# c-f-h/pyiga

Hardware: AMD Instinct MI355X
Metric: assembled elements/sec (3D p=4, 128^3 spans) + HBM-roofline %; 1/2/4/8 GPU (higher is better)
Workload: dtype f64

## Files before the change

### pyiga_amd/csrc/fused3.hip

```cpp
#include "igx_internal.h"
#include "fused_common.h"
#include <algorithm>
#include <cstdio>
#include <cstdlib>
#include <cstring>
#include <vector>

#ifndef BF3_FIXED_PASS
#define BF3_FIXED_PASS 1
#endif
#ifndef BF3_MASS_AXSYM
#define BF3_MASS_AXSYM 1
#endif
#ifndef BF3_MASS_STW
#define BF3_MASS_STW 1
#endif
#ifndef BF3_MASS_STW_QMAX
#define BF3_MASS_STW_QMAX 3
#endif

namespace igx {

template <int P1, int P2, int Q, int NLG, int NRO, int NCW, int SYM> struct BF3Geom {
    static constexpr int P1_ = P1, P2_ = P2, Q_ = Q;
    static constexpr int p1 = P1 - 1, p2 = P2 - 1, W1 = 2 * P1 - 1, W2 = 2 * P2 - 1, TL = 64 * NLG;
    static constexpr int NSET = SYM == 2 ? 2 : 1;
    static constexpr int QS = Q + (Q % 2 == 0 ? 1 : 0), NSP = (TL + Q - 1) / Q;
    static constexpr int TLP = TL + NSP * (QS - Q);
    static constexpr int VS = Q * P2 * 2 + ((Q * P2 * 2) % 4 == 2 ? 0 : 2), NV2 = NSP * VS;
    static constexpr int LS = NRO * TLP + 2;
    static constexpr int NRING = p1 * (p1 + 1) / 2 + p1;
    static constexpr int NRL = NRING + P1;
    static constexpr int T0 = p2 * (p2 + 1) / 2;
    static constexpr int NEL = 2 * p2 * W2;
    static constexpr int off_sets() { return (W1 * LS + 1) & ~1; }
    static constexpr int off_v2(int R) { return (off_sets() + NSET * (NRL * R * W2 + 2) + 1) & ~1; }
    static constexpr int off_etab(int R) { return off_v2(R) + NV2; }
    static constexpr int lds_doubles(int R) { return off_etab(R) + NEL * 2; }
    static constexpr int rmax()
    {
        int R = TL / Q - p2;
        while (R > 1 && lds_doubles(R) * 8 > 160 * 1024) --R;
        return R;
    }
    static constexpr int RMAX = rmax();
    static constexpr int RW = RMAX * W2;
    static constexpr int SETSZ = NRL * RW + 2;
    static constexpr int OFF_PAD = NRL * RW;
    static constexpr int roff(int d) { return RW * ((d - 1) * (d + 2) / 2); }
    static constexpr int OFF_CUR = NRING * RW;
    static constexpr int OFF_SETS = off_sets(), OFF_V2 = off_v2(RMAX), OFF_ETAB = off_etab(RMAX);
    static constexpr int LDS_BYTES = lds_doubles(RMAX) * 8;
    static constexpr int NSUB = (RW + 63) / 64;
    static constexpr int npc(int pl) { return (RMAX + pl - p2 - 1) / (pl - p2); }
    static constexpr int npass(int pl) { return (W1 * npc(pl) + 64 / pl - 1) / (64 / pl); }
    static constexpr int pick()
    {
        int best = 64;
        const int cand[4] = {64, 32, 21, 16};
        for (int i = 1; i < 4; ++i)
            if (cand[i] > 2 * p2 && npass(cand[i]) < npass(best)) best = cand[i];
        return best;
    }
    static constexpr int PL = pick(), PPP = 64 / PL, NPC = npc(PL), RP = PL - p2;
};

struct BF3Blk {
    int i0, j0, diag0, c0i, c0j, cj0, ci0, rlo, rhi, row_lo, nrows, stD, stT, ne;
    long long S12;
};

typedef int bf3_v4i __attribute__((ext_vector_type(4)));

template <class Gm> struct BF3Row {
    int on, l0, c1, rp1d, sub1, sub2, sub3, sub4, sub5;
    __device__ __forceinline__ static BF3Row of(const BFArgs &A, const BF3Blk &B, const int t)
    {
        cip rp1 = (cip)A.rp1, jlo1 = (cip)A.jlo1, jhi1 = (cip)A.jhi1;
        constexpr int p1 = Gm::p1, RW = Gm::RW;
        BF3Row r;
        const int d = t - 1;
        r.on = d >= B.rlo && d < B.rhi;
        const int dc = min(max(d, 0), A.N1 - 1);
        const int jl1 = jlo1[dc];
        r.c1 = jhi1[dc] - jl1; r.l0 = p1 - (dc - jl1);
        r.rp1d = rp1[dc];
        r.sub1 = Gm::roff(1) + (int)((unsigned)dc % 2u) * RW; r.sub2 = Gm::roff(2) + (int)((unsigned)dc % 3u) * RW;
        r.sub3 = Gm::roff(3) + (int)((unsigned)dc % 4u) * RW; r.sub4 = Gm::roff(4) + (int)((unsigned)dc % 5u) * RW;
        r.sub5 = Gm::roff(5) + (int)((unsigned)dc % 6u) * RW;
        return r;
    }
    __device__ __forceinline__ int line_off(const int l) const
    {
        constexpr int p1 = Gm::p1;
        int o = Gm::OFF_CUR + (l - p1) * Gm::RW;
        o = l == p1 - 1 ? sub1 : o;
        if (p1 >= 2) o = l == p1 - 2 ? sub2 : o;
        if (p1 >= 3) o = l == p1 - 3 ? sub3 : o;
        if (p1 >= 4) o = l == p1 - 4 ? sub4 : o;
        if (p1 >= 5) o = l == p1 - 5 ? sub5 : o;
        return o;
    }
    __device__ __forceinline__ bool line_ok(const int l) const { return l < Gm::W1 && l >= l0 && l - l0 < c1; }
};
__device__ __forceinline__ __amdgpu_buffer_rsrc_t bf3_rs(double *ptr, const int len) { return __builtin_amdgcn_make_buffer_rsrc((void *)ptr, (short)0, len, 0x00020000); }

template <class Gm, int NS, int ROT, int NH, int SYM, bool TR>
struct BF3Store {
    static constexpr int P1 = Gm::P1_, W1 = Gm::W1, W2 = Gm::W2, p2 = Gm::p2, NSUB = Gm::NSUB, RW = Gm::RW;
    static constexpr int JMAX = (W1 + NS - 1) / NS, NST = NSUB * JMAX, NSET = SYM == 2 ? 2 : 1;
    using Row = BF3Row<Gm>;
    int rrv[NSUB];
    int ev[TR ? NSUB : 1];
    int lane8, lanec, inv;
    double *pD, *pT;
    int nD, nT;

    __device__ __forceinline__ void init(const BFArgs &A, const BF3Blk &B, const int , const int lane)
    {
        cip rp0 = (cip)A.rp0;
        lane8 = lane * 8;
        lanec = min((NSUB - 1) * 64 + lane, RW - 1) - (NSUB - 1) * 64;
        if constexpr (TR) {
            pD = A.data + ((long long)rp0[B.i0] * B.S12 - A.nnz_off); nD = B.stD ? (int)((long long)B.c0i * B.S12 * 8) : 0;
            pT = A.data + ((long long)rp0[B.j0] * B.S12 - A.nnz_off); nT = B.stT ? (int)((long long)B.c0j * B.S12 * 8) : 0;
            inv = 2 * (int)A.S2 + 1;
#pragma unroll
            for (int c = 0; c < NSUB; ++c) {
                const int q = c * 64 + lane, rr = q / W2, i2 = B.row_lo + rr;
                const bool ok = q < RW && rr < B.nrows && i2 >= p2 && i2 <= A.N2 - 1 - p2;
                rrv[c] = ok ? W2 * i2 - Gm::T0 : inv;
                ev[c] = 8 * (q - rr * W2);
            }
            return;
        }
        const long long shift = (long long)W2 * B.row_lo - Gm::T0;
        const long long lenD = ((long long)B.c0i * B.S12 - shift) * 8, lenT = ((long long)B.c0j * B.S12 - shift) * 8;
        pD = A.data + ((long long)rp0[B.i0] * B.S12 - A.nnz_off + shift); nD = B.stD ? (int)lenD : 0;
        pT = A.data + ((long long)rp0[B.j0] * B.S12 - A.nnz_off + shift); nT = B.stT ? (int)lenT : 0;
        const int c0min = min(B.c0i, B.c0j);
        inv = (int)(max(lenD, lenT) / (8 * max(c0min * 2 - 1, 1))) + 1;
#pragma unroll
        for (int c = 0; c < NSUB; ++c) {
            const int q = c * 64 + lane, rr = q / W2, i2 = B.row_lo + rr;
            const bool ok = q < RW && rr < B.nrows && i2 >= p2 && i2 <= A.N2 - 1 - p2;
            rrv[c] = ok ? W2 * i2 - Gm::T0 : inv;
        }
    }
    __device__ __forceinline__ static int line_of(const int sw, const int c, const int j) { return (int)((unsigned)(sw + ROT * c) % (unsigned)NS) + NS * j; }

    template <int X>
    __device__ __forceinline__ void move_row(double *sets, double *dump, const int sw, const int lane, const Row &r, double *ptr, const int len, const int sK, const int soff0)
    {
        int lb_ = lane, lc_ = lanec;
        asm volatile("" : "+v"(lb_), "+v"(lc_));
        double *bs = sets + X * Gm::SETSZ + lb_, *bc = sets + X * Gm::SETSZ + (NSUB - 1) * 64 + lc_;
        double v[NST];
#pragma unroll
        for (int c = 0; c < NSUB; ++c)
#pragma unroll
            for (int j = 0; j < JMAX; ++j) {
                const int l = line_of(sw, c, j);
                double *src = (c == NSUB - 1 ? bc : bs + c * 64) + r.line_off(min(l, W1 - 1));
                v[c * JMAX + j] = *src;
                if (NH >= 2) {
                    double *cl = (rrv[c] != inv && l < W1) ? src : dump;
                    *cl = 0.0;
                }
            }
#ifdef BF3_NOSTORE
        return;
#endif
        int voff[NSUB];
#pragma unroll
        for (int c = 0; c < NSUB; ++c) {
            if constexpr (TR) voff[c] = (int)(__umul24((unsigned)rrv[c], (unsigned)sK) + __umul24((unsigned)ev[c], (unsigned)r.c1));
            else voff[c] = (int)__umul24((unsigned)rrv[c], (unsigned)sK) + lane8;
            asm volatile("" : "+v"(voff[c]));
        }
#pragma unroll
        for (int c = 0; c < NSUB; ++c)
#pragma unroll
            for (int j = 0; j < JMAX; ++j) {
                const int l = line_of(sw, c, j);
                if constexpr (TR) bf2_buffer_store(bf3_rs(ptr, r.line_ok(l) ? len : 0), voff[c], soff0 + 8 * l, v[c * JMAX + j]);
                else bf2_buffer_store(bf3_rs(ptr, r.line_ok(l) ? len : 0), voff[c] + c * 512, soff0 + 8 * W2 * l, v[c * JMAX + j]);
            }
    }
    __device__ __forceinline__ void fetch(const BFArgs &A, const BF3Blk &B, double *sets, double *dump, const int t, const int sw, const int lane)
    {
        const Row r = Row::of(A, B, t);
        if constexpr (TR) {
            const int sD = 8 * B.c0i * (int)A.S1, sT = 8 * B.c0j * (int)A.S1;
            const int oD = 8 * (W2 * (B.c0i * r.rp1d + B.cj0 * r.c1) - r.l0), oT = 8 * (W2 * (B.c0j * r.rp1d + B.ci0 * r.c1) - r.l0);
            move_row<0>(sets, dump, sw, lane, r, pD, r.on ? nD : 0, sD, oD);
            if (NSET == 2) move_row<1>(sets, dump, sw, lane, r, pT, r.on ? nT : 0, sT, oT);
            if (SYM == 3) move_row<0>(sets, dump, sw, lane, r, pT, r.on ? nT : 0, sT, oT);
            return;
        }
        move_row<0>(sets, dump, sw, lane, r, pD, r.on ? nD : 0, 8 * (B.c0i * r.c1 - 1), 8 * ((int)((long long)B.c0i * A.S2) * r.rp1d + W2 * (B.cj0 * r.c1 - r.l0)));
        if (NSET == 2)
            move_row<1>(sets, dump, sw, lane, r, pT, r.on ? nT : 0, 8 * (B.c0j * r.c1 - 1), 8 * ((int)((long long)B.c0j * A.S2) * r.rp1d + W2 * (B.ci0 * r.c1 - r.l0)));
        if (SYM == 3)
            move_row<0>(sets, dump, sw, lane, r, pT, r.on ? nT : 0, 8 * (B.c0j * r.c1 - 1), 8 * ((int)((long long)B.c0j * A.S2) * r.rp1d + W2 * (B.ci0 * r.c1 - r.l0)));
    }
};

template <int NR, int NLG, int NQ> struct BF3DenseSplit {
    static constexpr int NA = (NR - 2) * NLG, NB = NLG;
    static constexpr int ka() { if (NA == 0) return 0; int k = 1; while (NA * k + NB * ((3 * k + 1) / 2) < NQ) ++k; return k; }
    static constexpr int KA = ka(), KB = NA == 0 ? (NQ + NB - 1) / NB : (3 * KA + 1) / 2;
    static constexpr int QB = NA * KA < NQ ? NA * KA : NQ;
};
constexpr int BF3_FAR = 0x7f000000;
template <class Gm, int NH, int SYM, int K, int QLO, int QHI, int QSTR, bool TR>
struct BF3StoreDense {
    static constexpr int p1 = Gm::p1, p2 = Gm::p2, W1 = Gm::W1, W2 = Gm::W2, WW = W1 * W2, RW = Gm::RW, NSET = SYM == 2 ? 2 : 1;
    using Row = BF3Row<Gm>;
    double svD[K], svT[NSET == 2 ? K : 1];
    int pk[K];
    int lane8;
    double *pD, *pT;
    long long nD, nT;

    __device__ __forceinline__ void init(const BFArgs &A, const BF3Blk &B, const int sw, const int lane)
    {
        cip rp0 = (cip)A.rp0;
        lane8 = lane * 8;
        pD = A.data + ((long long)rp0[B.i0] * B.S12 - A.nnz_off); nD = B.stD ? (long long)B.c0i * B.S12 * 8 : 0;
        pT = A.data + ((long long)rp0[B.j0] * B.S12 - A.nnz_off); nT = B.stT ? (long long)B.c0j * B.S12 * 8 : 0;
#pragma unroll
        for (int k = 0; k < K; ++k) {
            svD[k] = 0.0;
            if (NSET == 2) svT[k] = 0.0;
            const int qi = QLO + sw + QSTR * k;
            const int q = qi * 64 + lane, rr = q / WW, rem = q - rr * WW, l = rem / W2, e = rem - l * W2, i2 = B.row_lo + rr;
            const bool ok = qi < QHI && q < Gm::RMAX * WW && rr < B.nrows && i2 >= p2 && i2 <= A.N2 - 1 - p2;
            pk[k] = ok ? (4 * l) | ((rr * W2 + e) << 6) | (rr << 18) : (int)(0x80000000u | 60u);
        }
    }

    __device__ __forceinline__ void fetch(const BFArgs &A, const BF3Blk &B, double *sets, double *dump, const int t, const int sw, const int lane)
    {
        const Row r = Row::of(A, B, t);
        int lv = Gm::OFF_CUR + (lane - p1) * RW;
        lv = lane == p1 - 1 ? r.sub1 : lv;
        if (p1 >= 2) lv = lane == p1 - 2 ? r.sub2 : lv;
        if (p1 >= 3) lv = lane == p1 - 3 ? r.sub3 : lv;
        if (p1 >= 4) lv = lane == p1 - 4 ? r.sub4 : lv;
        if (p1 >= 5) lv = lane == p1 - 5 ? r.sub5 : lv;
        lv = lane == 15 ? Gm::OFF_PAD : lv;
#pragma unroll
        for (int k = 0; k < K; ++k) {
            int pkk = pk[k];
            asm volatile("" : "+v"(pkk));
            const int lo = __builtin_amdgcn_ds_bpermute(pkk & 60, lv) + ((pkk >> 6) & 0xfff);
            double *src = sets + lo;
            svD[k] = *src;
#ifndef BF3_NOCLEAR
            if (NH >= 2) *src = 0.0;
#endif
            if (NSET == 2) {
                double *srcT = src + Gm::SETSZ;
                svT[k] = *srcT;
#ifndef BF3_NOCLEAR
                if (NH >= 2) *srcT = 0.0;
#endif
            }
        }
        (void)dump;
    }

    __device__ __forceinline__ void issue(const BFArgs &A, const BF3Blk &B, const int t, const int sw)
    {
#ifdef BF3_NOSTORE
        return;
#endif
        const Row r = Row::of(A, B, t);
        if constexpr (TR) {
            const long long rowc = (long long)W2 * B.row_lo - Gm::T0;
            const long long shD = (long long)B.c0i * A.S1 * rowc + (long long)W2 * (B.c0i * r.rp1d + B.cj0 * r.c1) - r.l0;
            const long long shT = (long long)B.c0j * A.S1 * rowc + (long long)W2 * (B.c0j * r.rp1d + B.ci0 * r.c1) - r.l0;
            const __amdgpu_buffer_rsrc_t dD = bf3_rs(pD + shD, r.on ? (int)max(nD - shD * 8, 0LL) : 0);
            const __amdgpu_buffer_rsrc_t dT = bf3_rs(pT + shT, r.on ? (int)max(nT - shT * 8, 0LL) : 0);
            const int dlD = 8 * W2 * (B.c0i * (int)A.S1 - r.c1), dlT = 8 * W2 * (B.c0j * (int)A.S1 - r.c1), c18 = 8 * r.c1;
            const int lane = lane8 >> 3;
            const int offl = (unsigned)(lane - r.l0) < (unsigned)r.c1 ? lane8 : BF3_FAR;
#pragma unroll
            for (int k = 0; k < K; ++k) {
                int pkk = pk[k];
                asm volatile("" : "+v"(pkk));
                const int rr = (pkk >> 18) & 0xff;
                const int q8 = __builtin_amdgcn_ds_bpermute(pkk & 60, offl) + (int)__mul24((pkk >> 6) & 0xfff, c18);
                bf2_buffer_store(dD, (int)__mul24(rr, dlD) + q8, 0, svD[k]);
                if (NSET == 2) bf2_buffer_store(dT, (int)__mul24(rr, dlT) + q8, 0, svT[k]);
                if (SYM == 3) bf2_buffer_store(dT, (int)__mul24(rr, dlT) + q8, 0, svD[k]);
            }
            return;
        }
        const int cD = B.c0i * r.c1, cT = B.c0j * r.c1;
        const long long rowc = (long long)W2 * B.row_lo - Gm::T0;
        const long long shD = (long long)B.c0i * A.S2 * r.rp1d + cD * rowc + W2 * (B.cj0 * r.c1 - r.l0);
        const __amdgpu_buffer_rsrc_t dD = bf3_rs(pD + shD, r.on ? (int)max(nD - shD * 8, 0LL) : 0);
        const int dlD = 8 * W2 * (cD - W1);
        const long long shT = (long long)B.c0j * A.S2 * r.rp1d + cT * rowc + W2 * (B.ci0 * r.c1 - r.l0);
        const __amdgpu_buffer_rsrc_t dT = bf3_rs(pT + shT, r.on ? (int)max(nT - shT * 8, 0LL) : 0);
        const int dlT = 8 * W2 * (cT - W1);
        const int lane = lane8 >> 3;
        const int offl = (unsigned)(lane - r.l0) < (unsigned)r.c1 ? 0 : BF3_FAR;
#pragma unroll
        for (int k = 0; k < K; ++k) {
            int pkk = pk[k];
            asm volatile("" : "+v"(pkk));
            const int rr = (pkk >> 18) & 0xff;
            const int q8 = __builtin_amdgcn_ds_bpermute(pkk & 60, offl) + ((QLO + sw + QSTR * k) * 512 + lane8);
            bf2_buffer_store(dD, (int)__mul24(rr, dlD) + q8, 0, svD[k]);
            if (NSET == 2) bf2_buffer_store(dT, (int)__mul24(rr, dlT) + q8, 0, svT[k]);
            if (SYM == 3) bf2_buffer_store(dT, (int)__mul24(rr, dlT) + q8, 0, svD[k]);
        }
    }
};

template <class Gm, int NCW, int NH, int SYM, bool TR>
__device__ __forceinline__ void bf3_edge_rows(const BFArgs &A, const BF3Blk &B, double *sets, const bf3_v4i *etab, const int t, const int cw, const int lane)
{
    constexpr int W1 = Gm::W1, W2 = Gm::W2;
    if (B.ne == 0) return;
    cip rp0 = (cip)A.rp0;
    const BF3Row<Gm> r = BF3Row<Gm>::of(A, B, t);
    const long long shift = (long long)W2 * B.row_lo - Gm::T0;
    static_assert(SYM != 3 || NH == 1, "per-axis symmetry: the second store reads the rows again (no halves, no clears)");
#pragma unroll
    for (int X = 0; X < (SYM == 3 ? 2 : Gm::NSET); ++X) {
        if (X == 0 ? !B.stD : !B.stT) continue;
        const int c0x = X == 0 ? B.c0i : B.c0j, cx = X == 0 ? B.cj0 : B.ci0;
        double *px = A.data + ((long long)rp0[X == 0 ? B.i0 : B.j0] * B.S12 - A.nnz_off + (TR ? 0 : shift));
        const int nx = (int)(((long long)c0x * B.S12 - (TR ? 0 : shift)) * 8);
        const unsigned sA = TR ? (unsigned)(c0x * r.rp1d + cx * r.c1) : (unsigned)(c0x * r.c1);
        const unsigned sC = (unsigned)(8 * c0x * (int)A.S1);
        const int soffr = TR ? 0 : 8 * (int)((long long)c0x * A.S2) * r.rp1d;
        for (int l = (int)((unsigned)(cw + NCW - X) % (unsigned)NCW); l < W1; l += NCW) {
            const unsigned sB = TR ? (unsigned)r.c1 : (unsigned)max(cx * r.c1 + l - r.l0, 0);
            const __amdgpu_buffer_rsrc_t dsc = bf3_rs(px, (r.on && r.line_ok(l)) ? nx : 0);
            double *lb = sets + (SYM == 3 ? 0 : X) * Gm::SETSZ + r.line_off(l);
            for (int ch = 0; ch * 64 < B.ne * W2; ++ch) {
                const bf3_v4i e = etab[min(ch * 64 + lane, Gm::NEL - 1)];
                const bool ok = ch * 64 + lane < Gm::NEL && e.w != BF2_OOB;
                double *src = lb + e.x;
                const double v = *src;
                if (NH >= 2 && ok) *src = 0.0;
                int off = (int)(__umul24(sA, (unsigned)e.y) + __umul24(sB, (unsigned)e.z));
                if constexpr (TR) off += (int)__umul24(sC, (unsigned)e.w) + 8 * (l - r.l0);
                else off += e.w;
                bf2_buffer_store(dsc, ok ? off : BF2_OOB, soffr, v);
            }
        }
    }
}

struct BF3SweepCtx { const BF3Blk *B; double *sets, *dump; int sw, tlp; };
template <int P1, int Q, int D, int MASK, int RI, int NA, int NLG, class StoreT, bool STW, bool MULT>
__device__ __forceinline__ void bf3_sweeper(const BFArgs &A, const int r0, const int g2l, const int g2, const int s_begin, const int t_sw, const int d_begin,
                                            const int rhi, double *lines, const int LS, const BF3SweepCtx &sc)
{
    constexpr BFRole R = bf_role(MASK, RI);
    constexpr int p1 = P1 - 1;
    constexpr bool ST = STW && (RI >= 1 || bf_nroles(MASK) == 1);
    const int slane = threadIdx.x & 63;
    StoreT store;
    if constexpr (ST) store.init(A, *sc.B, sc.sw, slane);
    BF_STAMP_DECL
    __builtin_amdgcn_s_setprio(BF2_PRIO_S);
    cdp V1 = (cdp)A.V1;
    cip fa1 = (cip)A.fa1;
    double acc[P1][P1];
#pragma unroll
    for (int a = 0; a < P1; ++a)
#pragma unroll
        for (int b = 0; b < P1; ++b) acc[a][b] = 0.0;
    __amdgpu_buffer_rsrc_t rsrc[4][NA];
    int urs[4][NA];
    const int voff = g2 * 8;
#pragma unroll
    for (int t1 = 0; t1 < 4; ++t1)
#pragma unroll
        for (int i = 0; i < NA; ++i) {
            urs[t1][i] = A.rs[R.y][t1][i] * 8;
            rsrc[t1][i] = bf2_rsrc(A.sp[R.y][t1][i] + (long long)r0 * A.ss[R.y][t1][i] - (long long)A.gmid_lo * A.rs[R.y][t1][i]);
        }
    auto ld = [&](const int t1, const int i, const int row) {
#ifdef BF3_NOLOAD
        return (double)(row + t1);
#else
        return bf2_buffer_load(rsrc[t1][i], voff, row * urs[t1][i]);
#endif
    };
    static_assert(Q % D == 0, "k_bf3: the prefetch ring must divide the span");
    double kv[D][4][NA];
    {
        const int s = min(s_begin, max(t_sw - 1, 0));
#pragma unroll
        for (int l = 0; l < D; ++l)
#pragma unroll
            for (int t1 = 0; t1 < 4; ++t1)
                if (R.has[t1])
#pragma unroll
                    for (int i = 0; i < NA; ++i) kv[l][t1][i] = ld(t1, i, s * Q + l);
    }
    auto flush = [&](const bool zero) {
        double *ln = lines + RI * sc.tlp + g2l;
#pragma unroll
        for (int a = 0; a < P1; ++a) ln[a * LS] = acc[a][0];
#pragma unroll
        for (int a = 1; a < P1; ++a) ln[(p1 + a) * LS] = acc[0][a];
#pragma unroll
        for (int a = 0; a < P1 - 1; ++a)
#pragma unroll
            for (int b = 0; b < P1 - 1; ++b) acc[a][b] = acc[a + 1][b + 1];
        if (zero) {
#pragma unroll
            for (int a = 0; a < P1; ++a) { acc[a][P1 - 1] = 0.0; acc[P1 - 1][a] = 0.0; }
        }
    };
    auto sweep_span = [&](const int s) __attribute__((always_inline)) {
        const int tn = min(s + 1, t_sw - 1);
        cdp cf = V1 + (size_t)s * Q * P1 * 2;
        double v[P1][2];
#pragma unroll
        for (int b = 0; b < P1; ++b) { v[b][0] = cf[2 * b]; v[b][1] = cf[2 * b + 1]; }
#pragma unroll
        for (int l = 0; l < Q; ++l) {
            double vn[P1][2];
            const int ln_ = l + 1 < Q ? l + 1 : l;
#pragma unroll
            for (int b = 0; b < P1; ++b) { vn[b][0] = cf[(ln_ * P1 + b) * 2]; vn[b][1] = cf[(ln_ * P1 + b) * 2 + 1]; }
            double kt[4] = {0.0, 0.0, 0.0, 0.0};
#pragma unroll
            for (int t1 = 0; t1 < 4; ++t1)
                if (R.has[t1]) {
                    kt[t1] = kv[l % D][t1][0];
                    if constexpr (NA == 2) kt[t1] += kv[l % D][t1][1];
#pragma unroll
                    for (int i = 0; i < NA; ++i) kv[l % D][t1][i] = ld(t1, i, l + D < Q ? s * Q + l + D : tn * Q + l + D - Q);
                }
            if (R.shape == 1) {
#pragma unroll
                for (int b = 0; b < P1; ++b) {
                    double w;
                    if (R.has[2 * R.f] && R.has[2 * R.f + 1]) w = fma(v[b][1], kt[2 * R.f + 1], v[b][0] * kt[2 * R.f]);
                    else if (R.has[2 * R.f]) w = v[b][0] * kt[2 * R.f];
                    else w = v[b][1] * kt[2 * R.f + 1];
#pragma unroll
                    for (int a = 0; a < P1; ++a) {
                        if (l == 0 && (a == P1 - 1 || b == P1 - 1)) acc[a][b] = v[a][R.f] * w;
                        else acc[a][b] = fma(v[a][R.f], w, acc[a][b]);
                    }
                }
            } else {
                constexpr int tu_first = (R.has[0] || R.has[2]) ? 0 : 1;
#pragma unroll
                for (int tu = 0; tu < 2; ++tu) {
                    if (!(R.has[tu] || R.has[tu + 2])) continue;
#pragma unroll
                    for (int a = 0; a < P1; ++a) {
                        double c;
                        if (R.has[tu] && R.has[tu + 2]) c = fma(v[a][1], kt[tu + 2], v[a][0] * kt[tu]);
                        else if (R.has[tu]) c = v[a][0] * kt[tu];
                        else c = v[a][1] * kt[tu + 2];
#pragma unroll
                        for (int b = 0; b < P1; ++b) {
                            if (l == 0 && tu == tu_first && (a == P1 - 1 || b == P1 - 1)) acc[a][b] = v[b][tu] * c;
                            else acc[a][b] = fma(v[b][tu], c, acc[a][b]);
                        }
                    }
                }
            }
#pragma unroll
            for (int a = 0; a < P1; ++a)
#pragma unroll
                for (int b = 0; b < P1; ++b) asm volatile("" : "+v"(acc[a][b]));
#pragma unroll
            for (int b = 0; b < P1; ++b) { v[b][0] = vn[b][0]; v[b][1] = vn[b][1]; }
        }
    };
    if constexpr (!MULT) {
        int d = d_begin;
        for (; d < t_sw; ++d) {
            bar_lds();
            if constexpr (ST) store.issue(A, *sc.B, d - 1, sc.sw);
            sweep_span(d);
            bar_lds();
            flush(d + 1 >= t_sw);
            if constexpr (ST) store.fetch(A, *sc.B, sc.sets, sc.dump, d, sc.sw, slane);
        }
        for (; d < rhi; ++d) {
            bar_lds();
            if constexpr (ST) store.issue(A, *sc.B, d - 1, sc.sw);
            bar_lds(); flush(true);
            if constexpr (ST) store.fetch(A, *sc.B, sc.sets, sc.dump, d, sc.sw, slane);
        }
    } else {
        int s = s_begin;
        for (int d = d_begin; d < rhi; ++d) {
            bar_lds();
            if constexpr (ST) store.issue(A, *sc.B, d - 1, sc.sw);
            if (s < t_sw && fa1[s] == d) { sweep_span(s); ++s; }
            bar_lds();
            flush(true);
            if constexpr (ST) store.fetch(A, *sc.B, sc.sets, sc.dump, d, sc.sw, slane);
        }
    }
    {
        bar_lds();
        if constexpr (ST) store.issue(A, *sc.B, rhi - 1, sc.sw);
        bar_lds();
        if constexpr (ST) store.fetch(A, *sc.B, sc.sets, sc.dump, rhi, sc.sw, slane);
    }
    if constexpr (ST) store.issue(A, *sc.B, rhi, sc.sw);
    BF_STAMP_END(threadIdx.x >> 6);
}

template <int P1, int Q, int D, int MASK, int NA, int NLG, class StoreA, class StoreB, bool STW, bool MULT, int RI, bool END = (RI >= bf_nroles(MASK))>
struct BF3SweepDispatch {
    __device__ static __forceinline__ void run(const BFArgs &A, int role, int r0, int g2l, int g2, int s_begin, int t_sw, int d_begin, int rhi, double *lines, int LS, const BF3SweepCtx &sc)
    {
        if (role == RI) {
            if constexpr (RI == bf_nroles(MASK) - 1) bf3_sweeper<P1, Q, D, MASK, RI, NA, NLG, StoreB, STW, MULT>(A, r0, g2l, g2, s_begin, t_sw, d_begin, rhi, lines, LS, sc);
            else bf3_sweeper<P1, Q, D, MASK, RI, NA, NLG, StoreA, STW, MULT>(A, r0, g2l, g2, s_begin, t_sw, d_begin, rhi, lines, LS, sc);
        } else BF3SweepDispatch<P1, Q, D, MASK, NA, NLG, StoreA, StoreB, STW, MULT, RI + 1>::run(A, role, r0, g2l, g2, s_begin, t_sw, d_begin, rhi, lines, LS, sc);
    }
};
template <int P1, int Q, int D, int MASK, int NA, int NLG, class StoreA, class StoreB, bool STW, bool MULT, int RI>
struct BF3SweepDispatch<P1, Q, D, MASK, NA, NLG, StoreA, StoreB, STW, MULT, RI, true> {
    __device__ static __forceinline__ void run(const BFArgs &, int, int, int, int, int, int, int, int, double *, int, const BF3SweepCtx &) {}
};

struct BF3Unit {
    const double *lines, *V2s;
    double *sets;
    int dd, rlo, rhi, nhi, row_lo, nrows, lane, npieces;
    int diag0, stD, stT;
    int rbs1, rbs2, rbs3, rbs4, rbs5;
};
template <class Gm, int NY, int MASK, int SYM, int H>
__device__ __forceinline__ void bf3_unit(const BF3Unit U, const int pass)
{
    constexpr int P2 = Gm::P2_, Q = Gm::Q_, p1 = Gm::p1, p2 = Gm::p2, W1 = Gm::W1, W2 = Gm::W2;
    constexpr int TL = Gm::TL, LS = Gm::LS, RW = Gm::RW, PL = Gm::PL, PPP = Gm::PPP, NPC = Gm::NPC, RP = Gm::RP;
    constexpr int AH = (P2 + 1) / 2;
    constexpr int A0 = H == 2 ? AH : 0, A1 = H == 1 ? AH : P2;
    const int lane = U.lane, dd = U.dd;
    int ln_ = min(lane, PPP * PL - 1);
    asm volatile("" : "+v"(ln_));
    const int ps = ln_ / PL, x = ln_ - ps * PL;
    const int pid = pass * PPP + ps;
    const int k9 = pid / NPC, pj = pid - k9 * NPC;
    const int s1 = pj * RP + x;
    const bool colt = k9 <= p1;
    const int la = colt ? k9 : k9 - p1;
    const int row1 = colt ? dd + la : dd, col1 = colt ? dd : dd + la;
    const double *kl = U.lines + min(k9, W1 - 1) * LS + min(s1, TL / Q - 1) * Gm::QS, *vl = U.V2s + min(s1, TL / Q - 1) * Gm::VS;
    double loc[A1 - A0][P2];
#ifdef BF3_NOELEM
    {
        const double k0 = kl[0], v0 = vl[0];
#pragma unroll
        for (int a = 0; a < A1 - A0; ++a)
#pragma unroll
            for (int b = 0; b < P2; ++b) { loc[a][b] = k0 + v0 * (a + 3 * b); asm volatile("" : "+v"(loc[a][b])); }
    }
#else
    bf_element<P2, NY, MASK, A0, A1, Q>(loc, kl, vl, Gm::TLP);
#endif
    const int r3 = s1 - p2;
    const bool item = lane < PPP * PL && pid < U.npieces && x >= p2 && r3 < U.nrows && la < U.nhi;
    const int oshv = max(p2 - (U.row_lo + r3), 0);
    int rb = U.rbs1;
    if (p1 >= 2) rb = la == 2 ? U.rbs2 : rb;
    if (p1 >= 3) rb = la == 3 ? U.rbs3 : rb;
    if (p1 >= 4) rb = la == 4 ? U.rbs4 : rb;
    if (p1 >= 5) rb = la == 5 ? U.rbs5 : rb;
    const int cb = Gm::OFF_CUR + la * RW;
    if (U.stD) {
        double out[W2];
#pragma unroll
        for (int a = A0; a < A1; ++a)
#pragma unroll
            for (int b = 0; b < P2; ++b) {
                if (a == 0) out[b + p2] = loc[0][b];
                else if (a == A0 || b == 0) out[b - a + p2] = bf2_from_lane(((lane - a) & 63) * 4, loc[a - A0][b]);
                else out[b - a + p2] += bf2_from_lane(((lane - a) & 63) * 4, loc[a - A0][b]);
            }
        if (item && row1 >= U.rlo && row1 < U.rhi) {
            double *dste = U.sets + ((colt && la > 0) ? rb : cb) + r3 * W2 - oshv;
            constexpr int OLO = H == 0 ? 0 : p2 - (A1 - 1), OHI = H == 0 ? 2 * p2 : 2 * p2 - A0;
            if (SYM != 0 && U.diag0) {
                const int omax = la == 0 ? p2 : 2 * p2;
#pragma unroll
                for (int o = OLO; o <= OHI; ++o)
                    if (o >= oshv && o <= omax) {
                        if (H == 0) dste[o] = out[o];
                        else (void)__hip_atomic_fetch_add(dste + o, out[o], __ATOMIC_RELAXED, __HIP_MEMORY_SCOPE_WORKGROUP);
                    }
            } else if (H == 0) {
                if (U.row_lo >= p2) {
#pragma unroll
                    for (int o = 0; o < W2; ++o) dste[o] = out[o];
                } else {
#pragma unroll
                    for (int o = 0; o < W2; ++o)
                        if (o >= oshv) dste[o] = out[o];
                }
            } else {
                if (U.row_lo >= p2) {
#pragma unroll
                    for (int o = OLO; o <= OHI; ++o) {
                        if ((H == 1 && o > 2 * p2 - AH) || (H == 2 && o <= p2 - AH)) dste[o] = out[o];
                        else (void)__hip_atomic_fetch_add(dste + o, out[o], __ATOMIC_RELAXED, __HIP_MEMORY_SCOPE_WORKGROUP);
                    }
                } else {
#pragma unroll
                    for (int o = OLO; o <= OHI; ++o)
                        if (o >= oshv) {
                            if ((H == 1 && o > 2 * p2 - AH) || (H == 2 && o <= p2 - AH)) dste[o] = out[o];
                            else (void)__hip_atomic_fetch_add(dste + o, out[o], __ATOMIC_RELAXED, __HIP_MEMORY_SCOPE_WORKGROUP);
                        }
                }
            }
        }
    }
    __builtin_amdgcn_sched_barrier(0);
#pragma unroll
    for (int a = 0; a < A1 - A0; ++a)
#pragma unroll
        for (int b = 0; b < P2; ++b) asm volatile("" : "+v"(loc[a][b]));
    __builtin_amdgcn_sched_barrier(0);
#ifdef BF3_NOT
    if (SYM != 0 && U.diag0 && U.stD) {
#else
    if (SYM != 0 && (U.diag0 ? U.stD : U.stT)) {
#endif
        double outT[W2];
#pragma unroll
        for (int b = 0; b < P2; ++b)
#pragma unroll
            for (int a = A0; a < A1; ++a) {
                if (b == 0) outT[a + p2] = loc[a - A0][0];
                else if (a == A0) outT[a + p2 - b] = bf2_from_lane(((lane - b) & 63) * 4, loc[0][b]);
                else outT[a + p2 - b] += bf2_from_lane(((lane - b) & 63) * 4, loc[a - A0][b]);
            }
        if (item && col1 >= U.rlo && col1 < U.rhi) {
            constexpr int ELO = H == 0 ? 0 : A0, EHI = H == 0 ? 2 * p2 : A1 - 1 + p2;
            if (U.diag0) {
                double *dste = U.sets + cb + r3 * W2 - oshv;
                const int emin = la == 0 ? p2 + 1 : oshv;
#pragma unroll
                for (int e = ELO; e <= EHI; ++e)
                    if (e >= emin) {
                        if (H == 0) dste[e] = outT[e];
                        else (void)__hip_atomic_fetch_add(dste + e, outT[e], __ATOMIC_RELAXED, __HIP_MEMORY_SCOPE_WORKGROUP);
                    }
            } else {
                double *dste = U.sets + Gm::SETSZ + (colt ? cb : rb) + r3 * W2 - oshv;
                if (H == 0) {
                    if (U.row_lo >= p2) {
#pragma unroll
                        for (int e = 0; e < W2; ++e) dste[e] = outT[e];
                    } else {
#pragma unroll
                        for (int e = 0; e < W2; ++e)
                            if (e >= oshv) dste[e] = outT[e];
                    }
                } else if (U.row_lo >= p2) {
#pragma unroll
                    for (int e = ELO; e <= EHI; ++e) {
                        if ((H == 1 && e < AH) || (H == 2 && e >= p2 + AH)) dste[e] = outT[e];
                        else (void)__hip_atomic_fetch_add(dste + e, outT[e], __ATOMIC_RELAXED, __HIP_MEMORY_SCOPE_WORKGROUP);
                    }
                } else {
#pragma unroll
                    for (int e = ELO; e <= EHI; ++e)
                        if (e >= oshv) {
                            if ((H == 1 && e < AH) || (H == 2 && e >= p2 + AH)) dste[e] = outT[e];
                            else (void)__hip_atomic_fetch_add(dste + e, outT[e], __ATOMIC_RELAXED, __HIP_MEMORY_SCOPE_WORKGROUP);
                        }
                }
            }
        }
    }
}

template <int P1, int P2, int Q, int NY, int MASK, int NA, int NLG, int NCW, int NH, int SYM, bool MULT, bool TR = false>
__global__ void __launch_bounds__((bf_nroles(MASK) * NLG + NCW) * 64) k_bf3(const BFArgs A)
{
    using Gm = BF3Geom<P1, P2, Q, NLG, bf_nroles(MASK), NCW, SYM>;
    constexpr int p2 = P2 - 1, W1 = 2 * P1 - 1, W2 = 2 * P2 - 1, TL = Gm::TL, NR = bf_nroles(MASK), NSW = NR * NLG;
    constexpr int RW = Gm::RW, PPP = Gm::PPP, NPC = Gm::NPC;
    constexpr int LS = Gm::LS;
    extern __shared__ __attribute__((aligned(16))) double lds[];
    double *lines = lds;
    double *sets = lds + Gm::OFF_SETS;
    double *V2s = lds + Gm::OFF_V2;
    bf3_v4i *etab = (bf3_v4i *)(lds + Gm::OFF_ETAB);

    cip pl0 = (cip)A.pl0, jlo0 = (cip)A.jlo0, jhi0 = (cip)A.jhi0, fa1 = (cip)A.fa1, mslo1 = (cip)A.mslo1, jhi1 = (cip)A.jhi1;
    const int wave = __builtin_amdgcn_readfirstlane(threadIdx.x >> 6), lane = threadIdx.x & 63;
    unsigned bid = blockIdx.x;
    const bool tail = A.tail_k > 0 && bid >= A.main_blocks;
    {
        const unsigned per = (A.tail_k > 0 ? A.main_blocks : gridDim.x) / 8;
        if (bid < per * 8) bid = (bid % 8) * per + bid / 8;
    }
    int mch, mrows;
    if (tail) {
        const unsigned t = bid - A.main_blocks;
        mch = (int)(t % (unsigned)A.tail_k); mrows = A.tail_mrows;
        bid = A.main_blocks + t / (unsigned)A.tail_k;
    } else { mch = (int)((bid / A.ntiles) % A.nmchunks); mrows = A.mrows; }
    const int tile = (int)(bid % A.ntiles);
    const int r0 = (int)(bid / ((unsigned)A.ntiles * (tail ? 1 : A.nmchunks)));
    const int i0 = pl0[2 * r0], j0 = pl0[2 * r0 + 1];
    const bool diag0 = SYM != 0 && i0 == j0;
    const int row_lo = tile * A.R2, row_hi = min(row_lo + A.R2, A.N2), nrows = row_hi - row_lo;
    const int sp_lo = row_lo - p2;
    const int win0 = sp_lo * Q;
    const int rlo = A.mid_lo + mch * mrows, rhi = min(rlo + mrows, A.mid_hi);
    const int s_begin = mslo1[min(rlo, A.N1 - 1)];
    const int d_begin = fa1[s_begin];
    int t_sw = s_begin;
    {
        const int n_sw = min(A.n1, A.span_hi);
        while (t_sw < n_sw && fa1[t_sw] < rhi) ++t_sw;
    }

    for (int idx = threadIdx.x; idx < TL * P2 * 2; idx += blockDim.x) {
        const int gpt = win0 + idx / (2 * P2);
        const int pt = idx / (2 * P2), sp = pt / Q;
        V2s[sp * Gm::VS + (idx - sp * (Q * P2 * 2))] = (gpt >= 0 && gpt < A.G2) ? A.V2[(long long)win0 * P2 * 2 + idx] : 0.0;
    }
    if (NH >= 2)
        for (int idx = threadIdx.x; idx < Gm::OFF_V2 - Gm::OFF_SETS; idx += blockDim.x) sets[idx] = 0.0;
    const int lo_n = max(0, min(row_hi, min(p2, A.N2)) - row_lo);
    const int hi_s = max(max(p2, A.N2 - p2), row_lo), hi_n = max(0, row_hi - hi_s);
    const int ne = lo_n + hi_n;
    if (threadIdx.x < Gm::NEL) {
        const int k = threadIdx.x / W2, e = threadIdx.x - k * W2;
        bf3_v4i v; v.x = 0; v.y = 0; v.z = 0; v.w = BF2_OOB;
        if (k < ne) {
            const int i2 = k < lo_n ? row_lo + k : hi_s + (k - lo_n);
            const int jl2 = max(i2 - p2, 0), c2 = min(i2 + p2, A.N2 - 1) + 1 - jl2;
            if (e < c2) {
                const int shift = W2 * row_lo - Gm::T0;
                v.x = (i2 - row_lo) * W2 + e; v.y = 8 * A.rp2[i2]; v.z = 8 * c2; v.w = 8 * (e - shift);
                if constexpr (TR) { v.y = 8 * c2; v.z = 8 * e; v.w = A.rp2[i2]; }
            }
        }
        etab[threadIdx.x] = v;
    }

    int task = wave;
    if (NR == 4 && NLG == 2 && NCW == 8) {
        constexpr int tmap[16] = {0, 1, 2, 3, 6, 7, 4, 5, 8, 9, 10, 11, 12, 13, 14, 15};
        task = tmap[wave & 15];
    } else if (NR == 4 && NLG == 3 && NCW == 4) {
        constexpr int tmap[16] = {12, 13, 14, 15, 9, 3, 0, 2, 10, 4, 1, 7, 11, 6, 5, 8};
        task = tmap[wave & 15];
    } else if (NR == 4 && NLG == 2 && NCW == 4) {
        const int sd = wave & 3, k = wave >> 2;
        if (sd < 3) task = k == 0 ? NSW + sd : 2 * (sd + 1) + (k - 1);
        else task = k < 2 ? k : NSW + 3;
    }
    BF3Blk B;
    B.i0 = i0; B.j0 = j0; B.diag0 = diag0; B.c0i = jhi0[i0] - jlo0[i0]; B.c0j = jhi0[j0] - jlo0[j0];
    B.cj0 = j0 - jlo0[i0]; B.ci0 = i0 - jlo0[j0]; B.rlo = rlo; B.rhi = rhi;
    B.row_lo = row_lo; B.nrows = nrows; B.S12 = A.S1 * A.S2; B.ne = ne;
    B.stD = (i0 >= A.own_lo && i0 < A.own_hi) ? 1 : 0;
    B.stT = ((SYM == 2 || SYM == 3) && !diag0 && j0 >= A.own_lo && j0 < A.own_hi) ? 1 : 0;
    constexpr bool STW = NR >= 2 || (SYM == 3 && BF3_MASS_STW && Q <= BF3_MASS_STW_QMAX);
    constexpr int NQ = (Gm::RMAX * W1 * W2 + 63) / 64;
    using Split = BF3DenseSplit<NR < 2 ? 2 : NR, NLG, NQ>;
    using StoreA = BF3StoreDense<Gm, NH, SYM, Split::KA < 1 ? 1 : Split::KA, 0, Split::QB, Split::NA < 1 ? 1 : Split::NA, TR>;
    using StoreB = BF3StoreDense<Gm, NH, SYM, Split::KB, Split::QB, NQ, Split::NB, TR>;
    using StoreC = BF3Store<Gm, NCW, 1, NH, SYM, TR>;
    double *dump = lines + NR * Gm::TLP;
    if (task < NSW) {
        const int role = task / NLG, lg = task % NLG;
        const int g2l = lg * 64 + lane;
        const int g2 = min(max(win0 + g2l, 0), A.G2 - 1);
        const BF3SweepCtx sc{&B, sets, dump, role == NR - 1 ? lg : (role - 1) * NLG + lg, Gm::TLP};
        BF3SweepDispatch<P1, Q, (NH == 3 ? Q / 2 : Q), MASK, NA, NLG, StoreA, StoreB, STW, MULT, 0>::run(A, role, r0, g2l + (g2l / Q) * (Gm::QS - Q), g2, s_begin, t_sw, d_begin, rhi, lines, LS, sc);
        return;
    }

    const int cw = task - NSW;
    BF_STAMP_DECL
    __builtin_amdgcn_s_setprio(BF2_PRIO_C);
    StoreC store;
    if constexpr (!STW) store.init(A, B, cw, lane);
    const bool cdiag = diag0 || SYM == 3;
    const int nlines = cdiag ? P1 : W1;
    const int npieces = nlines * NPC;
    for (int t = d_begin; t < rhi + 1; ++t) {
        bar_lds();
        const int dd = t - 1;
        BF_SEG_BEGIN();
        if (dd >= d_begin && dd < rhi) {
            BF3Unit U;
            U.lines = lines; U.V2s = V2s; U.sets = sets; U.dd = dd; U.rlo = rlo; U.rhi = rhi; U.row_lo = row_lo; U.nrows = nrows;
            U.nhi = jhi1[dd] - dd;
            U.lane = lane; U.npieces = npieces; U.diag0 = cdiag; U.stD = SYM == 3 ? (B.stD | B.stT) : B.stD; U.stT = B.stT;
            U.rbs1 = Gm::roff(1) + (int)((unsigned)(dd + 1) % 2u) * RW; U.rbs2 = Gm::roff(2) + (int)((unsigned)(dd + 2) % 3u) * RW;
            U.rbs3 = Gm::roff(3) + (int)((unsigned)(dd + 3) % 4u) * RW; U.rbs4 = Gm::roff(4) + (int)((unsigned)(dd + 4) % 5u) * RW;
            U.rbs5 = Gm::roff(5) + (int)((unsigned)(dd + 5) % 6u) * RW;
            const int npass = (npieces + PPP - 1) / PPP;
            const int wslot = (int)((unsigned)(cw + t) % (unsigned)NCW);
            if constexpr (NH == 3) {
                for (int u = wslot; u < 2 * npass; u += NCW) {
                    if (u < npass) bf3_unit<Gm, NY, MASK, SYM, 2>(U, u);
                    else bf3_unit<Gm, NY, MASK, SYM, 1>(U, u - npass);
// ... 252 lines not shown
```

Before: 174.6 million.

## Rotate accumulator window by unrolling sweep steps and cache row state in store

The sweep loop is unrolled by P1 with a compile-time rotation index, so the sliding accumulator window is addressed modulo P1 instead of shifting P1^2 registers on every flush. The store helper now keeps the Row descriptor as a member computed once per step, and packs byte offsets directly into pk so fetch and issue need fewer shifts and multiplies. This is meant to cut per-step VALU register moves and index arithmetic. In exchange the code grows, the remainder loop still uses the copying flush, and the store keeps more live registers, which may affect occupancy.

```diff
diff --git a/pyiga_amd/csrc/fused3.hip b/pyiga_amd/csrc/fused3.hip
--- a/pyiga_amd/csrc/fused3.hip
+++ b/pyiga_amd/csrc/fused3.hip
@@ -220,13 +220,15 @@
     double svD[K], svT[NSET == 2 ? K : 1];
     int pk[K];
     int lane8;
+    Row r;
     double *pD, *pT;
     long long nD, nT;
 
-    __device__ __forceinline__ void init(const BFArgs &A, const BF3Blk &B, const int sw, const int lane)
+    __device__ __forceinline__ void init(const BFArgs &A, const BF3Blk &B, const int sw, const int lane, const int t0)
     {
         cip rp0 = (cip)A.rp0;
         lane8 = lane * 8;
+        r = Row::of(A, B, t0 - 1);
         pD = A.data + ((long long)rp0[B.i0] * B.S12 - A.nnz_off); nD = B.stD ? (long long)B.c0i * B.S12 * 8 : 0;
         pT = A.data + ((long long)rp0[B.j0] * B.S12 - A.nnz_off); nT = B.stT ? (long long)B.c0j * B.S12 * 8 : 0;
 #pragma unroll
@@ -236,13 +238,12 @@
             const int qi = QLO + sw + QSTR * k;
             const int q = qi * 64 + lane, rr = q / WW, rem = q - rr * WW, l = rem / W2, e = rem - l * W2, i2 = B.row_lo + rr;
             const bool ok = qi < QHI && q < Gm::RMAX * WW && rr < B.nrows && i2 >= p2 && i2 <= A.N2 - 1 - p2;
-            pk[k] = ok ? (4 * l) | ((rr * W2 + e) << 6) | (rr << 18) : (int)(0x80000000u | 60u);
-        }
-    }
-
-    __device__ __forceinline__ void fetch(const BFArgs &A, const BF3Blk &B, double *sets, double *dump, const int t, const int sw, const int lane)
-    {
-        const Row r = Row::of(A, B, t);
+            pk[k] = ok ? (4 * l) | ((rr * W2 + e) << 11) | (rr << 23) : (int)(0x80000000u | 60u);
+        }
+    }
+
+    __device__ __forceinline__ void fetch(double *sets, const int lane)
+    {
         int lv = Gm::OFF_CUR + (lane - p1) * RW;
         lv = lane == p1 - 1 ? r.sub1 : lv;
         if (p1 >= 2) lv = lane == p1 - 2 ? r.sub2 : lv;
@@ -250,12 +251,12 @@
         if (p1 >= 4) lv = lane == p1 - 4 ? r.sub4 : lv;
         if (p1 >= 5) lv = lane == p1 - 5 ? r.sub5 : lv;
         lv = lane == 15 ? Gm::OFF_PAD : lv;
+        lv *= 8;
 #pragma unroll
         for (int k = 0; k < K; ++k) {
-            int pkk = pk[k];
-            asm volatile("" : "+v"(pkk));
-            const int lo = __builtin_amdgcn_ds_bpermute(pkk & 60, lv) + ((pkk >> 6) & 0xfff);
-            double *src = sets + lo;
+            asm volatile("" : "+v"(pk[k]));
+            const int lo = __builtin_amdgcn_ds_bpermute(pk[k], lv) + (int)(((unsigned)pk[k] >> 8) & 0x7fffu);
+            double *src = (double *)((char *)sets + lo);
             svD[k] = *src;
 #ifndef BF3_NOCLEAR
             if (NH >= 2) *src = 0.0;
@@ -268,30 +269,32 @@
 #endif
             }
         }
-        (void)dump;
     }
 
     __device__ __forceinline__ void issue(const BFArgs &A, const BF3Blk &B, const int t, const int sw)
+    {
+        send(A, B, sw);
+        r = Row::of(A, B, t + 1);
+    }
+    __device__ __forceinline__ void send(const BFArgs &A, const BF3Blk &B, const int sw)
     {
 #ifdef BF3_NOSTORE
         return;
 #endif
-        const Row r = Row::of(A, B, t);
         if constexpr (TR) {
             const long long rowc = (long long)W2 * B.row_lo - Gm::T0;
             const long long shD = (long long)B.c0i * A.S1 * rowc + (long long)W2 * (B.c0i * r.rp1d + B.cj0 * r.c1) - r.l0;
             const long long shT = (long long)B.c0j * A.S1 * rowc + (long long)W2 * (B.c0j * r.rp1d + B.ci0 * r.c1) - r.l0;
             const __amdgpu_buffer_rsrc_t dD = bf3_rs(pD + shD, r.on ? (int)max(nD - shD * 8, 0LL) : 0);
             const __amdgpu_buffer_rsrc_t dT = bf3_rs(pT + shT, r.on ? (int)max(nT - shT * 8, 0LL) : 0);
-            const int dlD = 8 * W2 * (B.c0i * (int)A.S1 - r.c1), dlT = 8 * W2 * (B.c0j * (int)A.S1 - r.c1), c18 = 8 * r.c1;
+            const int dlD = 8 * W2 * (B.c0i * (int)A.S1 - r.c1), dlT = 8 * W2 * (B.c0j * (int)A.S1 - r.c1);
             const int lane = lane8 >> 3;
             const int offl = (unsigned)(lane - r.l0) < (unsigned)r.c1 ? lane8 : BF3_FAR;
 #pragma unroll
             for (int k = 0; k < K; ++k) {
-                int pkk = pk[k];
-                asm volatile("" : "+v"(pkk));
-                const int rr = (pkk >> 18) & 0xff;
-                const int q8 = __builtin_amdgcn_ds_bpermute(pkk & 60, offl) + (int)__mul24((pkk >> 6) & 0xfff, c18);
+                asm volatile("" : "+v"(pk[k]));
+                const int rr = (int)(((unsigned)pk[k] >> 23) & 0xffu);
+                const int q8 = __builtin_amdgcn_ds_bpermute(pk[k], offl) + (int)__mul24((int)(((unsigned)pk[k] >> 8) & 0x7fffu), r.c1);
                 bf2_buffer_store(dD, (int)__mul24(rr, dlD) + q8, 0, svD[k]);
                 if (NSET == 2) bf2_buffer_store(dT, (int)__mul24(rr, dlT) + q8, 0, svT[k]);
                 if (SYM == 3) bf2_buffer_store(dT, (int)__mul24(rr, dlT) + q8, 0, svD[k]);
@@ -310,10 +313,9 @@
         const int offl = (unsigned)(lane - r.l0) < (unsigned)r.c1 ? 0 : BF3_FAR;
 #pragma unroll
         for (int k = 0; k < K; ++k) {
-            int pkk = pk[k];
-            asm volatile("" : "+v"(pkk));
-            const int rr = (pkk >> 18) & 0xff;
-            const int q8 = __builtin_amdgcn_ds_bpermute(pkk & 60, offl) + ((QLO + sw + QSTR * k) * 512 + lane8);
+            asm volatile("" : "+v"(pk[k]));
+            const int rr = (int)(((unsigned)pk[k] >> 23) & 0xffu);
+            const int q8 = __builtin_amdgcn_ds_bpermute(pk[k], offl) + ((QLO + sw + QSTR * k) * 512 + lane8);
             bf2_buffer_store(dD, (int)__mul24(rr, dlD) + q8, 0, svD[k]);
             if (NSET == 2) bf2_buffer_store(dT, (int)__mul24(rr, dlT) + q8, 0, svT[k]);
             if (SYM == 3) bf2_buffer_store(dT, (int)__mul24(rr, dlT) + q8, 0, svD[k]);
@@ -359,6 +361,8 @@
 }
 
 struct BF3SweepCtx { const BF3Blk *B; double *sets, *dump; int sw, tlp; };
+template <int RT> struct BF3Rot { static constexpr int value = RT; };
+template <bool MV> struct BF3Move { static constexpr bool value = MV; };
 template <int P1, int Q, int D, int MASK, int RI, int NA, int NLG, class StoreT, bool STW, bool MULT>
 __device__ __forceinline__ void bf3_sweeper(const BFArgs &A, const int r0, const int g2l, const int g2, const int s_begin, const int t_sw, const int d_begin,
                                             const int rhi, double *lines, const int LS, const BF3SweepCtx &sc)
@@ -368,7 +372,7 @@
     constexpr bool ST = STW && (RI >= 1 || bf_nroles(MASK) == 1);
     const int slane = threadIdx.x & 63;
     StoreT store;
-    if constexpr (ST) store.init(A, *sc.B, sc.sw, slane);
+    if constexpr (ST) store.init(A, *sc.B, sc.sw, slane, d_begin);
     BF_STAMP_DECL
     __builtin_amdgcn_s_setprio(BF2_PRIO_S);
     cdp V1 = (cdp)A.V1;
@@ -407,22 +411,29 @@
 #pragma unroll
                     for (int i = 0; i < NA; ++i) kv[l][t1][i] = ld(t1, i, s * Q + l);
     }
-    auto flush = [&](const bool zero) {
+    auto flush = [&](const bool zero, auto rot, auto move) __attribute__((always_inline)) {
+        constexpr int RT = decltype(rot)::value;
+        constexpr bool MOVE = decltype(move)::value;
+        static_assert(!MOVE || RT == 0, "k_bf3: the copying flush works on the window at rest");
         double *ln = lines + RI * sc.tlp + g2l;
 #pragma unroll
-        for (int a = 0; a < P1; ++a) ln[a * LS] = acc[a][0];
-#pragma unroll
-        for (int a = 1; a < P1; ++a) ln[(p1 + a) * LS] = acc[0][a];
-#pragma unroll
-        for (int a = 0; a < P1 - 1; ++a)
-#pragma unroll
-            for (int b = 0; b < P1 - 1; ++b) acc[a][b] = acc[a + 1][b + 1];
+        for (int a = 0; a < P1; ++a) ln[a * LS] = acc[(a + RT) % P1][RT];
+#pragma unroll
+        for (int a = 1; a < P1; ++a) ln[(p1 + a) * LS] = acc[RT][(a + RT) % P1];
+        if constexpr (MOVE) {
+#pragma unroll
+            for (int a = 0; a < P1 - 1; ++a)
+#pragma unroll
+                for (int b = 0; b < P1 - 1; ++b) acc[a][b] = acc[a + 1][b + 1];
+        }
+        constexpr int NW = MOVE ? P1 - 1 : RT;
         if (zero) {
 #pragma unroll
-            for (int a = 0; a < P1; ++a) { acc[a][P1 - 1] = 0.0; acc[P1 - 1][a] = 0.0; }
+            for (int a = 0; a < P1; ++a) { acc[a][NW] = 0.0; acc[NW][a] = 0.0; }
         }
     };
-    auto sweep_span = [&](const int s) __attribute__((always_inline)) {
+    auto sweep_span = [&](const int s, auto rot) __attribute__((always_inline)) {
+        constexpr int RT = decltype(rot)::value;
         const int tn = min(s + 1, t_sw - 1);
         cdp cf = V1 + (size_t)s * Q * P1 * 2;
         double v[P1][2];
@@ -452,8 +463,9 @@
                     else w = v[b][1] * kt[2 * R.f + 1];
 #pragma unroll
                     for (int a = 0; a < P1; ++a) {
-                        if (l == 0 && (a == P1 - 1 || b == P1 - 1)) acc[a][b] = v[a][R.f] * w;
-                        else acc[a][b] = fma(v[a][R.f], w, acc[a][b]);
+                        double &ab = acc[(a + RT) % P1][(b + RT) % P1];
+                        if (l == 0 && (a == P1 - 1 || b == P1 - 1)) ab = v[a][R.f] * w;
+                        else ab = fma(v[a][R.f], w, ab);
                     }
                 }
             } else {
@@ -469,8 +481,9 @@
                         else c = v[a][1] * kt[tu + 2];
 #pragma unroll
                         for (int b = 0; b < P1; ++b) {
-                            if (l == 0 && tu == tu_first && (a == P1 - 1 || b == P1 - 1)) acc[a][b] = v[b][tu] * c;
-                            else acc[a][b] = fma(v[b][tu], c, acc[a][b]);
+                            double &ab = acc[(a + RT) % P1][(b + RT) % P1];
+                            if (l == 0 && tu == tu_first && (a == P1 - 1 || b == P1 - 1)) ab = v[b][tu] * c;
+                            else ab = fma(v[b][tu], c, ab);
                         }
                     }
                 }
@@ -484,37 +497,54 @@
         }
     };
     if constexpr (!MULT) {
-        int d = d_begin;
-        for (; d < t_sw; ++d) {
+        auto step = [&](const int d, auto rot) __attribute__((always_inline)) {
             bar_lds();
             if constexpr (ST) store.issue(A, *sc.B, d - 1, sc.sw);
-            sweep_span(d);
+            sweep_span(d, rot);
             bar_lds();
-            flush(d + 1 >= t_sw);
-            if constexpr (ST) store.fetch(A, *sc.B, sc.sets, sc.dump, d, sc.sw, slane);
+            flush(d + 1 >= t_sw, rot, BF3Move<false>{});
+            if constexpr (ST) store.fetch(sc.sets, slane);
+        };
+        int d = d_begin;
+        for (const int e = d_begin + (t_sw - d_begin) % P1; d < e; ++d) {
+            bar_lds();
+            if constexpr (ST) store.issue(A, *sc.B, d - 1, sc.sw);
+            sweep_span(d, BF3Rot<0>{});
+            bar_lds();
+            flush(d + 1 >= t_sw, BF3Rot<0>{}, BF3Move<true>{});
+            if constexpr (ST) store.fetch(sc.sets, slane);
+        }
+        for (; d < t_sw; d += P1) {
+            step(d, BF3Rot<0>{});
+            step(d + 1, BF3Rot<1>{});
+            if constexpr (P1 > 2) step(d + 2, BF3Rot<2>{});
+            if constexpr (P1 > 3) step(d + 3, BF3Rot<3>{});
+            if constexpr (P1 > 4) step(d + 4, BF3Rot<4>{});
+            if constexpr (P1 > 5) step(d + 5, BF3Rot<5>{});
+            static_assert(P1 >= 2 && P1 <= 6, "k_bf3: the unrolled step loop");
         }
         for (; d < rhi; ++d) {
             bar_lds();
             if constexpr (ST) store.issue(A, *sc.B, d - 1, sc.sw);
-            bar_lds(); flush(true);
-            if constexpr (ST) store.fetch(A, *sc.B, sc.sets, sc.dump, d, sc.sw, slane);
+            bar_lds(); flush(true, BF3Rot<0>{}, BF3Move<true>{});
+            if constexpr (ST) store.fetch(sc.sets, slane);
         }
     } else {
         int s = s_begin;
         for (int d = d_begin; d < rhi; ++d) {
             bar_lds();
             if constexpr (ST) store.issue(A, *sc.B, d - 1, sc.sw);
-            if (s < t_sw && fa1[s] == d) { sweep_span(s); ++s; }
+            if (s < t_sw && fa1[s] == d) { sweep_span(s, BF3Rot<0>{}); ++s; }
             bar_lds();
-            flush(true);
-            if constexpr (ST) store.fetch(A, *sc.B, sc.sets, sc.dump, d, sc.sw, slane);
+            flush(true, BF3Rot<0>{}, BF3Move<true>{});
+            if constexpr (ST) store.fetch(sc.sets, slane);
         }
     }
     {
         bar_lds();
         if constexpr (ST) store.issue(A, *sc.B, rhi - 1, sc.sw);
         bar_lds();
-        if constexpr (ST) store.fetch(A, *sc.B, sc.sets, sc.dump, rhi, sc.sw, slane);
+        if constexpr (ST) store.fetch(sc.sets, slane);
     }
     if constexpr (ST) store.issue(A, *sc.B, rhi, sc.sw);
     BF_STAMP_END(threadIdx.x >> 6);
```

Result: no change. 173.1 million (-0.8%).
